# xuanyi-fu/xynet

Hardware: AMD Instinct MI355X
Metric: GiB/s device-resident WebSocket XOR-unmask, 64KiB frames, 1/2/4/8 GPUs (higher is better)
Workload: dtype u8; 1 GPU; config 3: 32768 x 64 KiB masked binary frames (H=14), one contiguous 2 GiB batch; decoder=lattice (k_stream_lattice), mode=fused (xyws_decode_stream: boundaries discovered on device), frames_per_gpu=32768, batch_bytes_per_gpu=2147942400, payload_bytes_per_gpu=2147483648, batch_copies=1, parallelism=shard-by-frame x1, no collective

## Files before the change

### xynet_amd/_lib.py

```python
import ctypes as C
import os
import re

PKG = os.path.dirname(os.path.abspath(__file__))
ROOT = os.path.dirname(PKG)
HEADER = os.path.join(ROOT, "include", "xyws.h")

XYWS_OK = 0
XYWS_ERR_DEVICE = -5
OPT_PARSE_ONLY = 0x1
OPT_UNMASKED_HINT = 0x2
OPT_SERIAL_SCAN = 0x4
OPT_WG256 = 0x8
OPT_TEST_LATSPEC = 0x10
OPT_TEST_LATDUMP = 0x20
OPT_LATX_NOWORK = 0x40
OPT_LATX_ONLY = 0x80
OPT_STATS = 0x100
OPT_SMALL_SEG = 0x200
OPT_LATTICE = 0x400
OPT_NO_LATDEC = 0x800
OPT_NO_DENSE0 = 0x1000
OPT_REDIRECT = 0x2000
OPT_NO_LATENTRY = 0x4000
OPT_WG1024 = 0x8000
OPT_RUNS_NOWAIT = 0x10000
OPT_NO_STORE = 0x20000
OPT_WG512 = 0x40000
OPT_DIAG = 0x80000
OPT_TEST_GIVEUP = 0x100000
OPT_NO_LATTICE = 0x200000
OPT_STEAL = 0x400000
OPT_TEST_STEAL = 0x800000
OPT_LAT_NOGATE = 0x1000000
OPT_LAT_GATE = 0x2000000
OPT_BIGSCAN = 0x4000000
OPT_LATX_NOCHK = 0x8000000
OPT_IOV_PIECES = 0x10000000
OPT_IOV_STAGE = 0x20000000
OPT_NO_BIGSCAN = 0x40000000
OPT_RUNS = 0x80000000
NSTATS = 48
ST_RUNS, ST_NONE, ST_BAD, ST_REPAIR, ST_CUT, ST_SPIN, ST_SEGS, ST_FRAMES = 0, 1, 2, 3, 4, 5, 6, 7
ST_P_WIN, ST_P_CAND, ST_P_UND, ST_P_TCOMP, ST_P_TCHECK, ST_P_TRES = 8, 9, 10, 11, 12, 13
ST_D_TENT, ST_D_TCHASE = 14, 15
ST_T_PRO, ST_T_MAIN, ST_T_WAIT, ST_T_FILL, ST_T_CHASE, ST_T_XOR = 16, 17, 18, 19, 20, 21
ST_T_TAIL, ST_T_PF, ST_T_CP = 22, 23, 24
ST_P_FILL, ST_P_SCAN, ST_P_PUB, ST_D_NOENT, ST_D_CHASE, ST_D_MISMATCH, ST_D_OVF = 25, 26, 27, 28, 29, 30, 31
ST_GIVEUP, ST_BRIDGE, ST_STEAL_REQ, ST_STEAL_ACC, ST_STEAL_SEGS = 32, 33, 34, 35, 36
ST_D_TVAL, ST_T_ROWS, ST_T_SER = 37, 38, 39
ST_P_LATTICE, ST_X_W0, ST_X_BITS, ST_X_SURV, ST_T_STRIDE = 40, 41, 42, 43, 46
LT_C_A, LT_C_C, LT_C_ADV, LT_D_FILL, LT_D_WB, LT_D_TAB, LT_D_WC = 16, 17, 18, 19, 20, 21, 22
LT_D_MASK, LT_D_WD, LT_D_ST, LT_D_WA, LT_SEGS, LT_GATE, LT_END = 23, 24, 25, 26, 27, 28, 29
R_WORDS = 32
R_H, R_W, R_S0, R_HEAD, R_OKW, R_HN, R_WN, R_CNT, R_TAIL, R_FIRST, R_F0 = 0, 1, 2, 7, 8, 9, 10, 11, 12, 13, 14
R_EFROM, R_ECNT, R_EORD, R_ECARRY, R_EP = 20, 21, 22, 23, 24
R_T0, R_T1, R_T2, R_SPLIT, R_XCC, R_NREC = 25, 26, 27, 28, 29, 30
POL_EPOCH, POL_BYTES, POL_FSMIN, POL_FSMAX, POL_DECODER, POL_WORDS = 0, 1, 2, 3, 4, 5
DEC_RUNS, DEC_RUNS512, DEC_LATTICE = 0, 2, 3
DERR_TABLE, DERR_TIMEOUT, DERR_STALE, DERR_TAG, DERR_SRC_OOB, DERR_ORPHANS = 0x1, 0x2, 0x4, 0x8, 0x100, 0x200
ERRORS = {-1: "invalid argument", -2: "HIP runtime error", -3: "device allocation failed",
          -4: "scratch capacity exceeded", -5: "device-side error", -6: "not complete yet"}


class XywsError(RuntimeError):
    def __init__(self, code, what=""):
        self.code = code
        super().__init__(f"xyws error {code} ({ERRORS.get(code, '?')}){': ' + what if what else ''}")


class Frame(C.Structure):
    _fields_ = [("frame_off", C.c_int64), ("payload_off", C.c_int64),
                ("payload_len", C.c_uint64), ("key", C.c_uint8 * 4),
                ("flags", C.c_uint8), ("hdr_len", C.c_uint8),
                ("status", C.c_uint8), ("reserved", C.c_uint8)]


class Carry(C.Structure):
    _fields_ = [("payload_remaining", C.c_uint64), ("phase", C.c_uint64),
                ("frames_total", C.c_uint64), ("key", C.c_uint8 * 4),
                ("hdr_len", C.c_uint8), ("hdr", C.c_uint8 * 14),
                ("reserved", C.c_uint8 * 21)]


class Verdict(C.Structure):
    _fields_ = [("close_code", C.c_uint16), ("peer_code", C.c_uint16), ("action", C.c_uint8),
                ("reserved", C.c_uint8 * 3)]


class Message(C.Structure):
    _fields_ = [("first_frame", C.c_uint64), ("nframes", C.c_uint64), ("out_off", C.c_uint64),
                ("length", C.c_uint64), ("status", C.c_uint32), ("opcode", C.c_uint8),
                ("reserved", C.c_uint8 * 3)]


class MsgCarry(C.Structure):
    _fields_ = [("length", C.c_uint64), ("nframes", C.c_uint64), ("first_frame", C.c_uint64),
                ("frame_remaining", C.c_uint64), ("frames_seen", C.c_uint64), ("status", C.c_uint32),
                ("opcode", C.c_uint8), ("frame_member", C.c_uint8), ("utf8_len", C.c_uint8),
                ("utf8", C.c_uint8 * 3), ("reserved", C.c_uint8 * 14)]


class ArenaResult(C.Structure):
    _fields_ = [("seq", C.c_uint64), ("offset", C.c_uint64), ("len", C.c_uint64), ("nframes", C.c_uint64),
                ("frames", C.POINTER(Frame)), ("carry", Carry)]

# ... 155 lines not shown
```

### xynet_amd/csrc/xyws_lattice.h

```cpp

constexpr uint64_t LAT_FMIN = 128;
constexpr uint64_t LAT_FMAX = 1ull << 40;
enum { LS_AGG = 1, LS_BRK = 3 };
constexpr uint32_t LAT_SLIST = 512;
constexpr uint32_t LAT_NOCLAIM = 0x7FFFFFFFu;
enum : uint64_t { RD_DONE = 0, RD_FULL = 1, RD_FROM = 2 };

template <uint32_t NT_, uint32_t SEG_>
struct lgeom {
  static constexpr uint32_t NT = NT_, SEG = SEG_;
  static constexpr uint32_t TMAX = SEG_ / LAT_FMIN + 3;
};
using G_LAT = lgeom<1024, 15 * 8 * 1024>;
using G_LAT5 = lgeom<1024, 15 * 5 * 1024>;
constexpr uint64_t LAT5_MIN_FRAME = 16384;
using G_LAT_SMALL = lgeom<64, 1024>;


template <class GA, class GB>
struct llay {
  static_assert(GA::NT == GB::NT, "one workgroup size");
  static constexpr uint32_t NT = GA::NT;
  static constexpr uint32_t SEG = GA::SEG > GB::SEG ? GA::SEG : GB::SEG;
  static constexpr uint32_t TMAX = GA::TMAX > GB::TMAX ? GA::TMAX : GB::TMAX;
};
template <class GL>
struct __attribute__((aligned(256))) lat_lds {
  cstate S0;
  uint64_t E, X0, F, kmax, c0, kbf, nseg;
  uint64_t gk;
  uint32_t na, cur, nxt, brk, quit, done_last, nsl, big, nogate;
  uint64_t sl_seg[LAT_SLIST], sl_k[LAT_SLIST];
  uint4 tab[GL::TMAX];
  alignas(256) uint8_t seg[GL::SEG + 48];
};

XYWS_DEV uint32_t lat_rel(uint64_t x, uint64_t ss) {
  if (x <= ss) return 0;
  const uint64_t d = x - ss;
  return d > 0xFFFFFFFFull ? 0xFFFFFFFFu : (uint32_t)d;
}

constexpr uint32_t LAT_GRP = 64;
XYWS_DEV uint64_t lat_grp_size(const run_params& P, uint64_t g) {
  const uint64_t a = g * LAT_GRP;
  return a >= P.nseg ? 0 : (P.nseg - a < LAT_GRP ? P.nseg - a : LAT_GRP);
}

XYWS_DEV uint64_t lat_advance(const run_params& P, uint64_t E, uint32_t lane) {
  const uint64_t w = uniform64(st_load(P.lat + LW_W));
  if (w >= P.nseg) return w;
  uint64_t w1 = w;
  {
    const uint64_t g0 = w / LAT_GRP, g = g0 + lane, gs = lat_grp_size(P, g);
    const bool full = !gs || st_load(P.lgrp + g) == gs;
    const uint64_t nf = __ballot(!full);
    const uint32_t c = nf ? (uint32_t)__builtin_ctzll(nf) : 64u;
    const uint64_t wg = (g0 + c) * LAT_GRP;
    if (wg > w1) w1 = wg < P.nseg ? wg : P.nseg;
  }
  if (w1 < P.nseg) {
    bool dec[4];
#pragma unroll
    for (uint32_t r = 0; r < 4; r++) {
      const uint64_t j = w1 + 4 * lane + r;
      dec[r] = j >= P.nseg || (st_load(P.lat + LW_STAT + j) >> 2) == E;
    }
    const uint32_t lc = !dec[0] ? 0u : !dec[1] ? 1u : !dec[2] ? 2u : !dec[3] ? 3u : 4u;
    const uint64_t nd = __ballot(lc < 4);
    uint64_t w2 = w1 + 256;
    if (nd) {
      const uint32_t f = (uint32_t)__builtin_ctzll(nd);
      w2 = w1 + 4 * f + (uint32_t)__shfl((int)lc, (int)f, 64);
    }
    w1 = w2 < P.nseg ? w2 : P.nseg;
  }
  if (w1 > w && lane == 0) __hip_atomic_fetch_max(P.lat + LW_W, w1, __ATOMIC_RELAXED, __HIP_MEMORY_SCOPE_AGENT);
  return w1;
}
XYWS_DEV void lat_wait_decided(const run_params& P, uint64_t E, uint64_t s, uint32_t lane) {
  for (uint32_t it = 0; lat_advance(P, E, lane) <= s; it++) {
    if (it >= (1u << 20)) {
      if (lane == 0) atomicOr(head_error(P), DERR_TIMEOUT);
      return;
    }
    __builtin_amdgcn_s_sleep(8);
  }
}

XYWS_DEV u32x4 lat_mask(const uint4* tab, uint32_t nent, uint32_t idx, uint32_t a) {
  const uint4 g = tab[idx];
  if (g.x <= a && a + 16u <= g.y) return u32x4{g.z, g.z, g.z, g.z};
  u32x4 m = span_key16(a, g.x, g.y, g.z);
  if (idx + 1 < nent) {
    const uint4 n = tab[idx + 1];
    if (n.x < a + 16u) m |= span_key16(a, n.x, n.y, n.z);
  }
  return m;
}

XYWS_DEV hdr_info lat_hdr(const run_params& P, const uint8_t* seg, uint32_t xr, uint64_t x) {
  const uint32_t* q = reinterpret_cast<const uint32_t*>(seg + (xr & ~3u));
  const uint32_t sh = xr & 3u, r0 = q[0], r1 = q[1], r2 = q[2], r3 = q[3], r4 = q[4];
  uint32_t w[4];
  w[0] = __builtin_amdgcn_alignbyte(r1, r0, sh);
  w[1] = __builtin_amdgcn_alignbyte(r2, r1, sh);
  w[2] = __builtin_amdgcn_alignbyte(r3, r2, sh);
  w[3] = __builtin_amdgcn_alignbyte(r4, r3, sh);
  const uint64_t room = P.hi - x;
  return parse_header_words(w, room < 16 ? (uint32_t)room : 16u);
}

XYWS_DEV __amdgpu_buffer_rsrc_t lat_rsrc(const run_params& P, uint64_t ss, uint32_t n) {
  const uint64_t top = (P.hi + 15) & ~15ull;
  const uint64_t room = top > ss ? top - ss : 0;
  return __builtin_amdgcn_make_buffer_rsrc(P.base + ss, 0, room < n ? (uint32_t)room : n, 0x00020000);
}

XYWS_DEV void write_frame(const run_params& P, uint64_t ord, uint64_t start, const hdr_info& h, uint64_t ps,
                          int32_t hdr_shift);

XYWS_DEV void lat_carried_frame(const run_params& P, const xyws_carry* cz) {
  if (!P.frames || !P.cap || cz->payload_remaining || !cz->hdr_len) return;
  const hdr_info hh = header_carried(P, cz);
  if (hh.hlen) write_frame(P, 0, P.lo, hh, P.lo + (hh.hlen - cz->hdr_len), (int32_t)cz->hdr_len);
}

template <class LL>
XYWS_DEV void lat_finish(const run_params& P, LL& L) {
  uint64_t* rd = P.lat + LW_REDIR;
  const xyws_carry* cz = P.cin_user ? P.cin_user : &k_zero_carry;
  {
    const uint32_t w = L.na == 2 ? LW_NBAIL_POL : L.na ? LW_NBAIL_HYP : L.big ? LW_NLOOP_A : LW_NLOOP_B;
    st_store(P.lat + w, st_load(P.lat + w) + 1);
  }
  if (L.na) {
    st_store(rd, RD_FULL);
  } else {
    const uint64_t b = st_load(P.lat + LW_BRK);
    const uint64_t X0 = L.X0, F = L.F, kmax = L.kmax, c0 = L.c0;
    lat_carried_frame(P, cz);
    if (b) {
      const uint64_t kb = ~b;
      const uint64_t tb = c0 + kb;
      uint64_t* rc = P.lat + LW_RCARRY;
#pragma unroll
      for (int i = 0; i < 8; i++) st_store(rc + i, 0);
      st_store(rc + 2, cz->frames_total + tb);
      st_store(rd + 1, X0 + kb * F);
      st_store(rd + 2, tb);
      st_store(rd, RD_FROM);
    } else {
      const uint64_t xl = X0 + (kmax - 1) * F;
      const hdr_info h = hdr_global(P, xl, NONE);
      uint64_t total = c0 + kmax;
      cstate S;
      if (!h.hlen) {
        S.X = xl; S.cov_ps = xl; S.cov_start = xl; S.cov_kw = 0; S.cov_key = 0; S.st = S_PARTIAL | S_NOCOV; S.pad = 0;
        total--;
      } else {
        S = frame_state(xl, h);
      }
      xyws_carry cinc;
#pragma unroll
      for (int i = 0; i < 8; i++) reinterpret_cast<uint64_t*>(&cinc)[i] = reinterpret_cast<const uint64_t*>(cz)[i];
      write_outputs(P, &cinc, total, S);
      dpol_publish(P, F, DEC_LATTICE);
      if (P.pol) {
        const uint64_t v[5] = {L.E, P.hi - P.lo, F, F, DEC_LATTICE};
#pragma unroll
        for (int i = 1; i < 5; i++) __hip_atomic_store(P.pol + i, v[i], __ATOMIC_RELAXED, __HIP_MEMORY_SCOPE_SYSTEM);
        __hip_atomic_store(P.pol, v[0], __ATOMIC_RELEASE, __HIP_MEMORY_SCOPE_SYSTEM);
      }
      st_store(rd, RD_DONE);
    }
  }
  uint32_t* cnt = reinterpret_cast<uint32_t*>(P.lat + LW_CNT);
  st_store(P.lat + LW_BRK, 0);
  st_store(P.lat + LW_W, 0);
  st_store(P.lat + LW_LOOPS, 0);
  __hip_atomic_store(cnt, 0u, __ATOMIC_RELAXED, __HIP_MEMORY_SCOPE_AGENT);
  __hip_atomic_store(cnt + 1, 0u, __ATOMIC_RELAXED, __HIP_MEMORY_SCOPE_AGENT);
  st_store(P.lat + LW_EPOCH, L.E);
}

XYWS_DEV bool lat_redirect(run_params& P) {
  if (!(P.opts & XYWS_OPT_REDIRECT)) return true;
  const uint64_t* r = P.lat + LW_REDIR;
  const uint64_t st = uniform64(st_load(r));
  if (st == RD_DONE) return false;
  if (st != RD_FROM) return true;
  const uint64_t p = uniform64(st_load(r + 1)), tb = uniform64(st_load(r + 2));
  const uint64_t pal = p & ~15ull;
  P.obias = p - P.lo;
  P.base += pal;
  P.lo = p - pal;
  P.hi -= pal;
  const uint64_t seg = P.segb, nseg = (P.hi + seg - 1) / seg, maxr = P.nruns;
  P.rbytes = nseg <= maxr ? seg : ((P.hi + maxr - 1) / maxr + 15) & ~15ull;
  P.nruns = (uint32_t)((P.hi + P.rbytes - 1) / P.rbytes);
  P.nflat = 2 * P.nruns;
  P.cin_user = reinterpret_cast<const xyws_carry*>(P.lat + LW_RCARRY);
  P.tbias = tb;
  if (P.frames) {
    const uint64_t c = P.cap < tb ? P.cap : tb;
    P.frames += c;
    P.cap -= c;
  }
  return true;
}

template <class G>
struct lat_io {
  static constexpr bool CTRL = G::NT >= 256;
  static constexpr uint32_t NW = G::NT / 64, NDW = CTRL ? NW - 1 : NW;
  static constexpr uint32_t NROW = G::SEG / 1024, K = (NROW + NDW - 1) / NDW;
  static constexpr uint32_t CLAIM = CTRL ? 64u : 0u;
  static_assert(G::SEG % 1024 == 0, "segments are whole 1 KiB rows");
  XYWS_DEV static bool data_wave(uint32_t wave) { return !CTRL || wave != 0; }
  XYWS_DEV static uint32_t row(uint32_t wave, uint32_t k) { return (CTRL ? wave - 1 : wave) + NDW * k; }
  XYWS_DEV static bool valid(uint32_t wave, uint32_t k) { return K * NDW == NROW || row(wave, k) < NROW; }
};

XYWS_DEV uint64_t lat_load_late(const uint64_t* p) {
  uint64_t v;
  asm volatile("global_load_dwordx2 %0, %1, off sc1" : "=v"(v) : "v"(p) : "memory");
  return v;
}

constexpr uint32_t LAT_NREP = 64, LAT_REPW = 32;
inline constexpr uint64_t lat_rep_off(uint64_t segs) {
  return (LW_STAT + segs + segs / 64 + 1 + LAT_REPW - 1) / LAT_REPW * LAT_REPW;
}
inline constexpr uint64_t lat_sl_off(uint64_t segs) { return lat_rep_off(segs) + LAT_NREP * LAT_REPW; }
XYWS_DEV void lat_raise_brk(const run_params& P, uint64_t k, uint32_t lane) {
  uint64_t o = 0;
// ... 61 lines not shown
  constexpr uint32_t CW = IO::CLAIM / 64u;
  auto issue = [&](uint32_t s, bool claim, bool rows) {
    if constexpr (DT) {
      if (wave == CW) {
        if (lane == 0) {
          if (claim)
            asm volatile("global_atomic_add %0, %1, %2, off sc0" : "=v"(ahead) : "v"(cnt), "v"(1u) : "memory");
          else
            ahead = LAT_NOCLAIM;
        }
        cx = lat_ctrl_load(P, s, G::SEG, X0, F, kmax, tid);
      }
      if (rows) {
        const __amdgpu_buffer_rsrc_t rs = lat_rsrc(P, (uint64_t)s * G::SEG, G::SEG);
#pragma unroll
        for (uint32_t k = 0; k < IO::K; k++)
          e[k] = __builtin_amdgcn_raw_buffer_load_b128(rs, IO::valid(wave, k) ? lane * 16u : OOB,
                                                       IO::row(wave, k) * 1024u, AUX_NT);
      }
    }
  };
  if (DT && cur != NONE32) {
    const uint32_t a0 = ahead;
    issue(cur, false, true);
    ahead = a0;
    const __amdgpu_buffer_rsrc_t rs = lat_rsrc(P, (uint64_t)cur * G::SEG, G::SEG);
#pragma unroll
    for (uint32_t k = 0; k < IO::K; k++)
      __builtin_amdgcn_raw_buffer_store_b128(u32x4{0u, 0u, 0u, 0u}, rs, OOB, k * 1024u, AUX_ST_STREAM);
  }
  const uint32_t dl = IO::CTRL ? tid - 64u : tid, NDL = IO::NDW * 64u;
  while (cur != NONE32) {
    asm volatile("" : "+v"(tid));
    const uint64_t ss = (uint64_t)cur * G::SEG;
    const uint64_t se = ss + G::SEG;
    const uint64_t ka = ss <= X0 ? 0 : (ss - X0 + F - 1) / F;
    clk.mark(cl ? LT_C_ADV : LT_D_ST);
    __syncthreads();
    clk.mark(cl ? LT_C_ADV : LT_D_WA);
    if constexpr (DT) {
#pragma unroll
      for (uint32_t k = 0; k < IO::K; k++)
        if (IO::valid(wave, k)) *reinterpret_cast<u32x4*>(&L.seg[IO::row(wave, k) * 1024u + lane * 16u]) = e[k];
      if (clk.on) asm volatile("s_waitcnt lgkmcnt(0)" ::: "memory");
    }
    if (DT && wave == CW) {
      asm volatile("" : "+v"(ahead), "+v"(cx) : "v"(e[IO::K - 1].x));
      const uint32_t ln = tid & 63u;
      if (ln < 9) *reinterpret_cast<uint32_t*>(&L.seg[G::SEG + 4u * ln]) = cx;
      if (lane == 0) {
        const uint32_t a = ahead + 2u * gridDim.x;
        L.nxt = a < P.nseg ? a : NONE32;
        L.brk = NONE32;
      }
    }
    clk.mark(cl ? LT_C_A : LT_D_FILL);
    __syncthreads();
    clk.mark(cl ? LT_C_A : LT_D_WB);
    const uint32_t nxt = uniform32(L.nxt);
    uint64_t kz = se <= X0 ? 0 : (se - X0 + F - 1) / F;
    if (kz > kmax) kz = kmax;
    const uint32_t nl = kz > ka ? (uint32_t)(kz - ka) : 0u;
    if constexpr (DT) {
      if (tid == IO::CLAIM) {
        uint4 c = {0u, 0u, 0u, 0u};
        if (ka == 0) {
          const cstate S0 = L.S0;
          if (!(S0.st & S_NOCOV)) c = uint4{lat_rel(S0.cov_ps, ss), lat_rel(X0, ss), S0.cov_kw, 0u};
        } else if (ka <= kmax) {
          const uint64_t xc = X0 + (ka - 1) * F;
          const uint32_t sh = (uint32_t)(xc & 3);
          uint32_t w[4];
          const uint32_t* cw = reinterpret_cast<const uint32_t*>(&L.seg[G::SEG + 16]);
#pragma unroll
          for (int i = 0; i < 4; i++) w[i] = __builtin_amdgcn_alignbyte(cw[i + 1], cw[i], sh);
          const uint64_t room = P.hi - xc;
          const hdr_info h = parse_header_words(w, room < 16 ? (uint32_t)room : 16u);
          if (h.hlen) {
            const uint64_t ps = xc + h.hlen;
            const uint64_t end = ka == kmax ? sat_add(ps, h.plen) : xc + F;
            c = uint4{lat_rel(ps, ss), lat_rel(end < P.hi ? end : P.hi, ss), aligned_key(h.key, ps, 0), 0u};
          }
        }
        L.tab[0] = c;
      }
      if (nxt != NONE32) issue(nxt, !L.quit, true);
      const uint32_t nlw = (P.opts & XYWS_OPT_LATX_NOWORK) ? 0u : nl;
      for (uint32_t i = dl; i < nlw; i += NDL) {
        const uint64_t k = ka + i;
        const uint64_t x = X0 + k * F;
        const uint32_t xr = (uint32_t)(x - ss);
        const hdr_info h = lat_hdr(P, L.seg, xr, x);
        const bool last = k + 1 == kmax;
        const uint64_t fend = h.hlen ? sat_add(x + h.hlen, h.plen) : x;
        const bool ok = h.hlen ? ((uint64_t)h.hlen + h.plen == F && h.plen < F) || (last && fend >= P.hi) : last;
        if (!ok) atomicMin(&L.brk, i);
        uint4 en = {xr, xr, 0u, 0u};
        if (h.hlen) {
          const uint64_t ps = x + h.hlen;
          en = uint4{lat_rel(ps, ss), lat_rel(fend < P.hi ? fend : P.hi, ss), aligned_key(h.key, ps, 0), 0u};
        }
        L.tab[1 + i] = en;
      }
    }
    if (CT && tid == 0) {
      asm volatile("s_waitcnt vmcnt(0)" : "+v"(brk_seen)::"memory");
      if (cl) clk.mark(LT_GATE);
      L.gk = brk_seen;
    }
    clk.mark(cl ? LT_C_A : LT_D_TAB);
    __syncthreads();
    clk.mark(cl ? LT_C_C : LT_D_WC);
    const uint32_t brk = uniform32(L.brk);
    const bool blind = (P.opts & XYWS_OPT_TEST_LATSPEC) != 0;
    const bool gate = it == 0 && !blind && !(P.opts & XYWS_OPT_LAT_NOGATE);
    if (CT && tid < 64) {
      const uint64_t gk = uniform64(L.gk);
      if (brk != NONE32 && !(gk && ~gk <= ka + brk)) lat_raise_brk(P, ka + brk, lane);
      if (tid == 0) {
        st_store(P.lat + LW_STAT + cur, (E << 2) | (brk != NONE32 ? LS_BRK : LS_AGG));
        __hip_atomic_fetch_add(P.lgrp + cur / LAT_GRP, 1ull, __ATOMIC_RELAXED, __HIP_MEMORY_SCOPE_AGENT);
      }
      if (gate) {
        const uint64_t tg = clk.on ? __builtin_amdgcn_s_memtime() : 0;
        lat_wait_decided(P, E, cur, lane);
        if (tg && tid == 0) stat_add(P, LT_END, __builtin_amdgcn_s_memtime() - tg);
        if (tid == 0) L.gk = st_load(P.lat + LW_BRK);
      }
      if (tid == 0) brk_seen = lat_load_late(P.lbrk + LAT_REPW * (blockIdx.x % LAT_NREP));
    }
    if (gate) __syncthreads();
    clk.mark(cl ? LT_C_C : LT_D_WD);
    const uint64_t b = blind ? 0 : uniform64(L.gk);
    uint64_t kst = brk != NONE32 ? ka + brk : kz;
    if (b && ~b < kst) kst = ~b;
    uint32_t stop = kst >= kz ? G::SEG : lat_rel(X0 + kst * F, ss);
    if (stop > G::SEG) stop = G::SEG;
    bool quit = b || brk != NONE32;
    if (stop && !gate) {
      if (nsl < LAT_SLIST) {
        if (tid == IO::CLAIM) {
          L.sl_seg[nsl] = cur;
          L.sl_k[nsl] = kst;
        }
        nsl++;
      } else {
        const uint64_t k0 = ka ? ka - 1 : 0;
        if (tid == IO::CLAIM)
          for (uint32_t r = 0; r <= LAT_NREP; r++)
            __hip_atomic_fetch_max(r < LAT_NREP ? P.lbrk + LAT_REPW * r : P.lat + LW_BRK, ~k0, __ATOMIC_RELAXED,
                                   __HIP_MEMORY_SCOPE_AGENT);
        if (k0 < kst) {
          stop = lat_rel(X0 + k0 * F, ss);
          kst = k0;
        }
        quit = true;
      }
    }
    if (quit && tid == IO::CLAIM) L.quit = 1;
    if constexpr (DT) {
      const uint32_t xka = ka < kmax ? lat_rel(X0 + ka * F, ss) : 0xFFFFFFFFu;
      const uint32_t nent = brk != NONE32 ? 1u + brk : 1u + nl;
      const uint32_t lo_r = lat_rel(P.lo, ss), hi_r = P.hi - ss < G::SEG ? (uint32_t)(P.hi - ss) : G::SEG;
      const __amdgpu_buffer_rsrc_t rs = lat_rsrc(P, ss, G::SEG);
      const bool any = !(P.opts & XYWS_OPT_NO_STORE);
      const bool work = !(P.opts & XYWS_OPT_LATX_NOWORK);
      uint32_t edge = 0;
      u32x4 dprev = {0u, 0u, 0u, 0u};
#pragma unroll
      for (uint32_t k = 0; k < IO::K; k++) {
        const bool ok = IO::valid(wave, k);
        const uint32_t a = (ok ? IO::row(wave, k) : 0u) * 1024u + lane * 16u;
        u32x4 d = *reinterpret_cast<const u32x4*>(&L.seg[a]);
        uint32_t idx = 0;
// ... 75 lines not shown
        const cstate S0 = L.S0;
        if (!(S0.st & S_NOCOV)) en = uint4{lat_rel(S0.cov_ps, ss), lat_rel(X0, ss), S0.cov_kw, 0u};
      } else if (g < kst && g < kmax) {
        const uint64_t x = X0 + g * F;
        const hdr_info h = hdr_global(P, x, NONE);
        if (h.hlen) {
          const uint64_t ps = x + h.hlen;
          const uint64_t end = g + 1 == kmax ? sat_add(ps, h.plen) : x + F;
          en = uint4{lat_rel(ps, ss), lat_rel(end < P.hi ? end : P.hi, ss), aligned_key(h.key, ps, 0), 0u};
        }
      }
      m |= span_key16(a, en.x, en.y, en.z);
    }
    if (a >= from && a >= lo_r && a + 16u <= top) {
      uint32_t* q = reinterpret_cast<uint32_t*>(P.base + ss + a);
      const uint32_t mm[4] = {m.x, m.y, m.z, m.w};
#pragma unroll
      for (int i = 0; i < 4; i++) {
        if (!mm[i]) continue;
        const uint32_t v = __hip_atomic_load(q + i, __ATOMIC_RELAXED, __HIP_MEMORY_SCOPE_AGENT);
        __hip_atomic_store(q + i, v ^ mm[i], __ATOMIC_RELAXED, __HIP_MEMORY_SCOPE_AGENT);
      }
      continue;
    }
#pragma unroll
    for (uint32_t b = 0; b < 16; b++) {
      const uint32_t y = a + b;
      const uint32_t mw = b < 4 ? m.x : b < 8 ? m.y : b < 12 ? m.z : m.w;
      const uint8_t kbyte = (uint8_t)(mw >> (8u * (b & 3u)));
      if (kbyte && y >= from && y >= lo_r && y < top) {
        uint8_t* q = P.base + ss + y;
        const uint8_t v = __hip_atomic_load(q, __ATOMIC_RELAXED, __HIP_MEMORY_SCOPE_AGENT);
        __hip_atomic_store(q, (uint8_t)(v ^ kbyte), __ATOMIC_RELAXED, __HIP_MEMORY_SCOPE_AGENT);
      }
    }
  }
}

constexpr uint32_t LAT_UNDO_POLLS = 2048;

template <class G, class LL>
XYWS_DEV void lat_body(const run_params& P, LL& L, uint32_t tid, uint32_t ahead) {
  using IO = lat_io<G>;
  uint32_t* cnt = reinterpret_cast<uint32_t*>(P.lat + LW_CNT);
  if (!L.na) {
    if constexpr (IO::CTRL) {
      if (__builtin_amdgcn_readfirstlane(tid >> 6) == 0)
        lat_loop<G, LR_CTRL>(P, L, tid, ahead);
      else
        lat_loop<G, LR_DATA>(P, L, tid, ahead);
    } else {
      lat_loop<G, LR_ALL>(P, L, tid, ahead);
    }
    __syncthreads();
    if (tid < 64) {
      uint64_t b = 0;
      if (tid == 0) __hip_atomic_fetch_add(P.lat + LW_LOOPS, 1ull, __ATOMIC_RELAXED, __HIP_MEMORY_SCOPE_AGENT);
      if (L.quit && L.nsl) {
        const uint32_t polls = (P.opts & XYWS_OPT_TEST_LATDUMP) ? 0u : LAT_UNDO_POLLS;
        bool ended = false;
        for (uint32_t it = 0; it < polls; it++) {
          if (uniform64(st_load(P.lat + LW_LOOPS)) >= gridDim.x) {
            ended = true;
            break;
          }
          __builtin_amdgcn_s_sleep(8);
        }
        if (ended) b = uniform64(st_load(P.lat + LW_BRK));
      }
      if (tid == 0) L.kbf = b && L.nsl ? ~b : NONE;
    }
    __syncthreads();
    const uint64_t kb = L.kbf;
    if (kb != NONE) {
      const uint32_t n = L.nsl;
      for (uint32_t j = 0; j < n; j++)
        if (kb < L.sl_k[j]) lat_undo<G>(P, L, tid, L.sl_seg[j], L.sl_k[j], kb);
      asm volatile("s_waitcnt vmcnt(0)" ::: "memory");
      __syncthreads();
      if (tid == 0) L.nsl = 0;
      __syncthreads();
    }
    lat_dump_list<G>(P, L, tid);
  }
  asm volatile("s_waitcnt vmcnt(0)" ::: "memory");
  __syncthreads();
  if (tid == 0) {
    __builtin_amdgcn_fence(__ATOMIC_RELEASE, "agent");
    asm volatile("s_waitcnt vmcnt(0)" ::: "memory");
    const uint32_t last = atomicAdd(cnt + 1, 1u) + 1 == gridDim.x ? 1u : 0u;
    if (last) {
      __builtin_amdgcn_fence(__ATOMIC_ACQUIRE, "agent");
      asm volatile("s_waitcnt vmcnt(0)" ::: "memory");
    }
    L.done_last = last;
  }
  __syncthreads();
  if (!L.done_last) return;
  if (tid == 0) {
    const uint64_t b = st_load(P.lat + LW_BRK);
    L.kbf = b && !L.na ? ~b : NONE;
  }
  __syncthreads();
  const uint64_t kb = L.kbf;
  if (kb != NONE) {
    if (tid == 0) L.nsl = 0;
    __syncthreads();
    for (uint32_t w = tid; w < gridDim.x; w += G::NT) {
      const uint64_t* q = P.lsl + (uint64_t)w * LAT_LSW;
      const uint32_t n = (uint32_t)st_load(q);
      for (uint32_t i = 0; i < n; i++) {
        const uint64_t kst = st_load(q + 2 + 2 * i);
        if (kb < kst) {
          const uint32_t j = atomicAdd(&L.nsl, 1u);
          if (j < LAT_SLIST) {
            L.sl_seg[j] = st_load(q + 1 + 2 * i);
            L.sl_k[j] = kst;
          }
        }
      }
    }
    __syncthreads();
    const uint32_t nu = L.nsl;
    if (nu <= LAT_SLIST) {
      for (uint32_t j = 0; j < nu; j++) lat_undo<G>(P, L, tid, L.sl_seg[j], L.sl_k[j], kb);
    } else {
      for (uint32_t w = 0; w < gridDim.x; w++) {
        const uint64_t* q = P.lsl + (uint64_t)w * LAT_LSW;
        const uint32_t n = (uint32_t)st_load(q);
        for (uint32_t i = 0; i < n; i++) {
          const uint64_t kst = st_load(q + 2 + 2 * i);
          if (kb < kst) lat_undo<G>(P, L, tid, st_load(q + 1 + 2 * i), kst, kb);
        }
      }
    }
    asm volatile("s_waitcnt vmcnt(0)" ::: "memory");
    __syncthreads();
  }
  for (uint64_t g = tid; g * LAT_GRP < P.nseg; g += G::NT)
    __hip_atomic_store(P.lgrp + g, 0ull, __ATOMIC_RELAXED, __HIP_MEMORY_SCOPE_AGENT);
  if (tid < LAT_NREP) __hip_atomic_store(P.lbrk + LAT_REPW * tid, 0ull, __ATOMIC_RELAXED, __HIP_MEMORY_SCOPE_AGENT);
  if (tid != 0) return;
  lat_finish(P, L);
}

template <class GA, class GB>
__global__ void __launch_bounds__(GB::NT)
__attribute__((amdgpu_waves_per_eu(GB::NT >= 256 ? GB::NT / 256 : 1))) k_stream_lattice(run_params P0) {
  using GL = llay<GA, GB>;
  using IO = lat_io<GB>;
  static_assert(lat_io<GA>::CLAIM == IO::CLAIM, "one claim lane");
  extern __shared__ __attribute__((aligned(256))) uint8_t xs_lds[];
  lat_lds<GL>& L = *reinterpret_cast<lat_lds<GL>*>(xs_lds);
  const uint32_t tid = threadIdx.x;
  uint32_t ahead = NONE32;
  if (tid == 0) {
    const xyws_carry* cz = P0.cin_user ? P0.cin_user : &k_zero_carry;
    carry_words cc;
    uint32_t r0[5];
    uint64_t dp, ep;
    {
      u32x4 g;
      asm volatile("global_load_dwordx4 %0, %1, off sc1" : "=v"(g) : "v"(P0.lat + LW_DPOL) : "memory");
#pragma unroll
      for (int i = 0; i < 8; i++) cc.w[i] = reinterpret_cast<const uint64_t*>(cz)[i];
      const uint64_t a0 = P0.lo & ~3ull, dl = (P0.hi + 3) & ~3ull;
#pragma unroll
      for (int i = 0; i < 5; i++) {
        const uint64_t q = a0 + 4 * i;
        r0[i] = *reinterpret_cast<const uint32_t*>(P0.base + (q < dl ? q : dl - 4));
      }
      asm volatile("s_waitcnt vmcnt(0)" : "+v"(g)::"memory");
#pragma unroll
      for (int i = 0; i < 5; i++)
        if (a0 + 4 * i >= dl) r0[i] = 0u;
      dp = (uint64_t)g.x | ((uint64_t)g.y << 32);
      ep = (uint64_t)g.z | ((uint64_t)g.w << 32);
    }
    L.E = ep + 1;
    const bool dvalid = dp >> 63, dreg = (dp & ((1ull << 48) - 1)) >= LAT_FMIN;
    const uint64_t ddec = (dp >> 48) & 0x7Fu;
    uint32_t na = dvalid && !dreg && !(P0.opts & XYWS_OPT_LATTICE) ? 2u : 0u;
    L.nogate = dvalid && dreg && ddec == DEC_LATTICE && !(P0.opts & XYWS_OPT_LAT_GATE) ? 1u : 0u;
    uint64_t c0 = 0;
    const cstate S0 = initial_state_w(P0, cc, c0);
    if (!na && ((S0.st & S_PARTIAL) || S0.X >= P0.hi)) na = 1u;
    uint64_t F = 0, kmax = 0;
    if (!na) {
      hdr_info h;
      if (S0.X == P0.lo) {
        const uint32_t sh = (uint32_t)(P0.lo & 3);
        uint32_t w[4];
#pragma unroll
        for (int i = 0; i < 4; i++) w[i] = __builtin_amdgcn_alignbyte(r0[i + 1], r0[i], sh);
        const uint64_t room = P0.hi - P0.lo;
        h = parse_header_words(w, room < 16 ? (uint32_t)room : 16u);
      } else {
        h = hdr_global(P0, S0.X, NONE);
      }
      F = sat_add(h.hlen, h.plen);
      if (!h.hlen || F < LAT_FMIN || F > LAT_FMAX) na = 1;
      else kmax = (P0.hi - S0.X + F - 1) / F;
    }
    if (!na && kmax > 1 && !(P0.opts & (XYWS_OPT_TEST_LATSPEC | XYWS_OPT_LATX_NOCHK))) {
      const uint64_t dl = (P0.hi + 3) & ~3ull;
      uint32_t r[2][5];
#pragma unroll
      for (int j = 0; j < 2; j++) {
        const uint64_t a = (S0.X + (j + 1) * F) & ~3ull;
#pragma unroll
        for (int i = 0; i < 5; i++) {
          const uint64_t q = a + 4 * i;
          r[j][i] = (j == 0 || kmax > 2) && q < dl ? *reinterpret_cast<const uint32_t*>(P0.base + q) : 0u;
        }
      }
#pragma unroll
      for (int j = 0; j < 2; j++) {
        const uint64_t k = j + 1;
        if (k >= kmax) break;
        const uint64_t x = S0.X + k * F;
        const uint32_t sh = (uint32_t)(x & 3);
        uint32_t w[4];
#pragma unroll
        for (int i = 0; i < 4; i++) w[i] = __builtin_amdgcn_alignbyte(r[j][i + 1], r[j][i], sh);
        const uint64_t room = P0.hi - x;
        const hdr_info h = parse_header_words(w, room < 16 ? (uint32_t)room : 16u);
        const bool last = k + 1 == kmax;
        const uint64_t fend = h.hlen ? sat_add(x + h.hlen, h.plen) : x;
        const bool ok = h.hlen ? ((uint64_t)h.hlen + h.plen == F && h.plen < F) || (last && fend >= P0.hi) : last;
        if (!ok) na = 1;
      }
    }
    const bool big = GA::SEG != GB::SEG && !na && F >= LAT5_MIN_FRAME;
    const uint64_t seg = big ? GA::SEG : GB::SEG;
    const uint64_t nseg = (P0.hi + seg - 1) / seg;
    L.nseg = nseg;
    L.S0 = S0;
    L.c0 = c0;
    L.X0 = S0.X;
    L.F = F;
    L.kmax = kmax;
    L.na = na;
    L.quit = 0;
    L.nsl = 0;
    L.big = big ? 1u : 0u;
    L.cur = !na && blockIdx.x < nseg ? blockIdx.x : NONE32;
  }
  if (tid == IO::CLAIM) ahead = blockIdx.x - gridDim.x;
  __syncthreads();
  run_params P = P0;
  P.nseg = uniform64(L.nseg);
  P.opts &= ~XYWS_OPT_LAT_NOGATE;
  if (uniform32(L.nogate)) P.opts |= XYWS_OPT_LAT_NOGATE;
  if constexpr (GA::SEG != GB::SEG) {
    if (uniform32(L.big)) {
      lat_body<GA>(P, L, tid, ahead);
      return;
    }
  }
  lat_body<GB>(P, L, tid, ahead);
}
```

### xynet_amd/csrc/xyws_stream.h

```cpp
#pragma once
#include <hip/hip_runtime.h>
#include <stdint.h>
#include "xyws.h"
#include "xyws_host.h"


constexpr uint32_t HEAD_TICKET = 0;
constexpr uint32_t HEAD_ERROR = 4;
constexpr uint32_t HEAD_TOTAL = 8;
constexpr uint32_t HEAD_EPOCH = 16;
constexpr uint32_t HEAD_CARRY = 64;
constexpr uint32_t HEAD_STATS = 128;
constexpr uint32_t XYWS_NSTATS = 48;
constexpr uint32_t HW_DONE = 512;
constexpr uint32_t HW_BAD = 520;
constexpr uint32_t HW_TOTAL = 528;
constexpr uint32_t HW_FINAL = 536;
constexpr uint32_t HW_EMIT_SLOW = 584;
constexpr uint32_t HW_EMIT_FLAG = 592;
constexpr uint32_t HW_FSMAX = 600;
constexpr uint32_t HW_FSMIN = 608;
constexpr uint32_t HW_DPOL = 616;
constexpr uint32_t HEAD_BYTES = 1024;
static_assert(HEAD_CARRY + 64 <= HEAD_STATS && HEAD_STATS + 8 * XYWS_NSTATS <= HW_DONE, "head areas overlap");
// ... 13 lines not shown
  R_HEAD = 7,
  R_OKW = 8,
  R_HN = 9,
  R_WN = 10,
  R_CNT = 11,
  R_TAIL = 12,
  R_FIRST = 13,
  R_F0 = 14,
  R_EFROM = 20,
  R_ECNT = 21,
  R_EORD = 22,
  R_ECARRY = 23,
  R_EP = 24,
  R_T0 = 25,
  R_T1 = 26,
  R_T2 = 27,
  R_SPLIT = 28,
  R_XCC = 29,
  R_NREC = 30,
  R_WORDS = 32
};
static_assert(R_S0 + 5 == R_HEAD && R_F0 + 5 < R_EFROM && R_NREC < R_WORDS, "run record words overlap");

struct run_layout {
  uint64_t granules, split, prog, records;
  uint64_t zeroed, total;
};
inline run_layout run_layout_of(uint64_t units) {
  const auto pad = [](uint64_t bytes) { return (bytes + 255) & ~255ull; };
  run_layout l;
  l.granules = HEAD_BYTES;
  l.split = l.granules + pad(32 * units);
  l.prog = l.split + pad(16 * units);
  l.records = l.prog + pad(8 * units);
  l.zeroed = l.records;
  l.total = l.records + 2 * units * R_WORDS * 8;
  return l;
}

enum {
  LW_CNT = 0,
  LW_BRK = 2,
  LW_UNMASK = 3,
  LW_W = 4,
  LW_LOOPS = 5,
  LW_DPOL = 6,
  LW_EPOCH = 7,
  LW_REDIR = 8,
  LW_NBAIL_POL = 12,
  LW_NBAIL_HYP = 13,
  LW_NLOOP_A = 14,
  LW_NLOOP_B = 15,
  LW_RCARRY = 16,
  LW_STAT = 32
};
static_assert(LW_EPOCH == LW_DPOL + 1 && LW_DPOL % 2 == 0, "one 16-byte granule");

enum {
  ST_RUNS = 0,
  ST_NONE = 1,
  ST_BAD = 2,
  ST_REPAIR = 3,
  ST_CUT = 4,
  ST_SPIN = 5,
  ST_SEGS = 6,
  ST_FRAMES = 7,
  ST_P_WIN = 8,
  ST_P_CAND = 9,
  ST_P_UND = 10,
  ST_P_TCOMP = 11,
  ST_P_TCHECK = 12,
  ST_P_TRES = 13,
  ST_D_TENT = 14,
  ST_D_TCHASE = 15,
  ST_T_PRO = 16,
  LT_C_A = 16,
  ST_T_MAIN = 17,
  LT_C_C = 17,
  ST_T_WAIT = 18,
  LT_C_ADV = 18,
  ST_T_FILL = 19,
  LT_D_FILL = 19,
  ST_T_CHASE = 20,
  LT_D_WB = 20,
  ST_T_XOR = 21,
  LT_D_TAB = 21,
  ST_T_TAIL = 22,
  LT_D_WC = 22,
  ST_T_PF = 23,
  LT_D_MASK = 23,
  ST_T_CP = 24,
  LT_D_WD = 24,
  ST_P_FILL = 25,
  LT_D_ST = 25,
  ST_P_SCAN = 26,
  LT_D_WA = 26,
  ST_P_PUB = 27,
  LT_SEGS = 27,
  ST_D_NOENT = 28,
  LT_GATE = 28,
  ST_D_CHASE = 29,
  LT_END = 29,
  ST_D_MISMATCH = 30,
  ST_D_OVF = 31,
  ST_GIVEUP = 32,
  ST_BRIDGE = 33,
  ST_STEAL_REQ = 34,
  ST_STEAL_ACC = 35,
  ST_STEAL_SEGS = 36,
  ST_D_TVAL = 37,
  ST_T_ROWS = 38,
  ST_T_SER = 39,
  ST_P_LATTICE = 40,
  ST_X_W0 = 41,
  ST_X_BITS = 42,
  ST_X_SURV = 43,
  ST_T_STRIDE = 46
};
enum {
  LCLK_SLOT0 = 16,
  LCLK_NSLOTS = 16
};
static_assert(LT_C_A == LCLK_SLOT0 && LT_END < LCLK_SLOT0 + LCLK_NSLOTS && LCLK_SLOT0 + LCLK_NSLOTS <= ST_GIVEUP,
              "the lattice's clocks stay in the shared slots");
static_assert(ST_T_STRIDE < XYWS_NSTATS, "a stats slot outside the head's stats area");

enum {
  POL_EPOCH = 0,
  POL_BYTES = 1,
  POL_FSMIN = 2,
  POL_FSMAX = 3,
  POL_DECODER = 4,
  POL_WORDS = 5
};
enum : uint64_t {
  DEC_RUNS = 0,
  DEC_RUNS512 = 2,
  DEC_LATTICE = 3
};

constexpr uint64_t SCRATCH_MIN_RUNS = 64, SCRATCH_MIN_SEGS = 64;
struct stream_scratch {
  xyws_internal::dev_area runs;
  int ncu = 256;
  xyws_internal::dev_area desc;
  volatile uint64_t* pol_h = nullptr;
  uint64_t* pol_d = nullptr;
  xyws_internal::dev_area lat;
};

void stream_scratch_init(stream_scratch* s, int device);
void stream_scratch_free(stream_scratch* s);
int stream_scratch_reserve(stream_scratch* s, uint64_t max_batch_bytes, uint64_t max_frames);
uint32_t stream_scratch_error(stream_scratch* s, bool clear);
int stream_scratch_stats(stream_scratch* s, uint64_t out[XYWS_NSTATS]);
int64_t stream_scratch_records(stream_scratch* s, uint64_t* out, uint64_t max_runs);
int stream_scratch_lattice(stream_scratch* s, uint64_t out[5]);
int stream_scratch_unmask_counter(stream_scratch* s, bool capturing, uint32_t** out);

#define XYWS_OPT_WG256 0x8u
#define XYWS_OPT_TEST_LATSPEC 0x10u
#define XYWS_OPT_TEST_LATDUMP 0x20u
#define XYWS_OPT_LATX_NOWORK 0x40u
#define XYWS_OPT_LATX_ONLY 0x80u
#define XYWS_OPT_STATS 0x100u
#define XYWS_OPT_SMALL_SEG 0x200u
#define XYWS_OPT_LATTICE 0x400u
#define XYWS_OPT_NO_LATDEC 0x800u
#define XYWS_OPT_NO_DENSE0 0x1000u
// ... 65 lines not shown
```

Baseline: 3075 GiB/s.

## Precompute last-frame carry state in segment workers to shorten lattice finish tail

The workgroup that handles the final segment now computes the last frame's carry state and writes it to a new tail record in scratch, tagged with the epoch. The finishing block loads the break word, the tail record and the input carry in one batch of loads. This lets it skip the global header re-read on its serial critical path, and the carried-frame write and outputs are moved after the bookkeeping stores. The atomic add for the loop counter and a reordered policy load trim a few more serialized round trips, at the cost of extra LDS state and a fallback path when the epoch tag does not match.

```diff
diff --git a/xynet_amd/_lib.py b/xynet_amd/_lib.py
--- a/xynet_amd/_lib.py
+++ b/xynet_amd/_lib.py
@@ -52,6 +52,7 @@
 ST_P_LATTICE, ST_X_W0, ST_X_BITS, ST_X_SURV, ST_T_STRIDE = 40, 41, 42, 43, 46
 LT_C_A, LT_C_C, LT_C_ADV, LT_D_FILL, LT_D_WB, LT_D_TAB, LT_D_WC = 16, 17, 18, 19, 20, 21, 22
 LT_D_MASK, LT_D_WD, LT_D_ST, LT_D_WA, LT_SEGS, LT_GATE, LT_END = 23, 24, 25, 26, 27, 28, 29
+LT_TAIL, LT_TAIL_FIN = 44, 45
 R_WORDS = 32
 R_H, R_W, R_S0, R_HEAD, R_OKW, R_HN, R_WN, R_CNT, R_TAIL, R_FIRST, R_F0 = 0, 1, 2, 7, 8, 9, 10, 11, 12, 13, 14
 R_EFROM, R_ECNT, R_EORD, R_ECARRY, R_EP = 20, 21, 22, 23, 24
diff --git a/xynet_amd/csrc/xyws_lattice.h b/xynet_amd/csrc/xyws_lattice.h
--- a/xynet_amd/csrc/xyws_lattice.h
+++ b/xynet_amd/csrc/xyws_lattice.h
@@ -24,12 +24,20 @@
   static constexpr uint32_t SEG = GA::SEG > GB::SEG ? GA::SEG : GB::SEG;
   static constexpr uint32_t TMAX = GA::TMAX > GB::TMAX ? GA::TMAX : GB::TMAX;
 };
+struct lat_fin {
+  uint64_t brk;
+  uint64_t rec[8];
+  xyws_carry cin;
+};
 template <class GL>
 struct __attribute__((aligned(256))) lat_lds {
   cstate S0;
   uint64_t E, X0, F, kmax, c0, kbf, nseg;
   uint64_t gk;
+  uint64_t ttail, tfin;
+  lat_fin fin;
   uint32_t na, cur, nxt, brk, quit, done_last, nsl, big, nogate;
+  uint32_t lastp;
   uint64_t sl_seg[LAT_SLIST], sl_k[LAT_SLIST];
   uint4 tab[GL::TMAX];
   alignas(256) uint8_t seg[GL::SEG + 48];
@@ -126,52 +134,75 @@
   if (hh.hlen) write_frame(P, 0, P.lo, hh, P.lo + (hh.hlen - cz->hdr_len), (int32_t)cz->hdr_len);
 }
 
+XYWS_DEV cstate lat_last_state(uint64_t xl, const hdr_info& h, uint64_t c0, uint64_t kmax, uint64_t& total) {
+  total = c0 + kmax;
+  if (h.hlen) return frame_state(xl, h);
+  cstate S;
+  S.X = xl; S.cov_ps = xl; S.cov_start = xl; S.cov_kw = 0; S.cov_key = 0; S.st = S_PARTIAL | S_NOCOV; S.pad = 0;
+  total--;
+  return S;
+}
+
+XYWS_DEV void lat_tail_put(const run_params& P, uint64_t E, const cstate& S, uint64_t total) {
+  uint64_t* r = P.lat + LW_TAIL;
+  put_state(r + 1, S);
+  st_store(r + 6, total);
+  st_store(r, E);
+}
+
+XYWS_DEV void lat_finish_load(const run_params& P, lat_fin& f) {
+  const xyws_carry* cz = P.cin_user ? P.cin_user : &k_zero_carry;
+  uint64_t c[8];
+#pragma unroll
+  for (int i = 0; i < 8; i++) c[i] = reinterpret_cast<const uint64_t*>(cz)[i];
+  uint64_t b;
+  u32x4 t0, t1, t2, t3;
+  asm volatile(
+      "global_load_dwordx2 %0, %5, off sc1\n\t"
+      "global_load_dwordx4 %1, %6, off sc1\n\t"
+      "global_load_dwordx4 %2, %6, off offset:16 sc1\n\t"
+      "global_load_dwordx4 %3, %6, off offset:32 sc1\n\t"
+      "global_load_dwordx4 %4, %6, off offset:48 sc1\n\t"
+      "s_waitcnt vmcnt(0)"
+      : "=&v"(b), "=&v"(t0), "=&v"(t1), "=&v"(t2), "=&v"(t3)
+      : "v"(P.lat + LW_BRK), "v"(P.lat + LW_TAIL)
+      : "memory");
+  f.brk = b;
+  const u32x4 t[4] = {t0, t1, t2, t3};
+#pragma unroll
+  for (int i = 0; i < 4; i++) {
+    f.rec[2 * i] = (uint64_t)t[i].x | ((uint64_t)t[i].y << 32);
+    f.rec[2 * i + 1] = (uint64_t)t[i].z | ((uint64_t)t[i].w << 32);
+  }
+#pragma unroll
+  for (int i = 0; i < 8; i++) reinterpret_cast<uint64_t*>(&f.cin)[i] = c[i];
+}
+
 template <class LL>
 XYWS_DEV void lat_finish(const run_params& P, LL& L) {
   uint64_t* rd = P.lat + LW_REDIR;
-  const xyws_carry* cz = P.cin_user ? P.cin_user : &k_zero_carry;
+  const xyws_carry* cz = &L.fin.cin;
   {
     const uint32_t w = L.na == 2 ? LW_NBAIL_POL : L.na ? LW_NBAIL_HYP : L.big ? LW_NLOOP_A : LW_NLOOP_B;
-    st_store(P.lat + w, st_load(P.lat + w) + 1);
-  }
+    __hip_atomic_fetch_add(P.lat + w, 1ull, __ATOMIC_RELAXED, __HIP_MEMORY_SCOPE_AGENT);
+  }
+  bool held = false;
   if (L.na) {
     st_store(rd, RD_FULL);
   } else {
-    const uint64_t b = st_load(P.lat + LW_BRK);
-    const uint64_t X0 = L.X0, F = L.F, kmax = L.kmax, c0 = L.c0;
-    lat_carried_frame(P, cz);
+    const uint64_t b = L.fin.brk;
     if (b) {
       const uint64_t kb = ~b;
-      const uint64_t tb = c0 + kb;
+      const uint64_t tb = L.c0 + kb;
       uint64_t* rc = P.lat + LW_RCARRY;
 #pragma unroll
       for (int i = 0; i < 8; i++) st_store(rc + i, 0);
       st_store(rc + 2, cz->frames_total + tb);
-      st_store(rd + 1, X0 + kb * F);
+      st_store(rd + 1, L.X0 + kb * L.F);
       st_store(rd + 2, tb);
       st_store(rd, RD_FROM);
     } else {
-      const uint64_t xl = X0 + (kmax - 1) * F;
-      const hdr_info h = hdr_global(P, xl, NONE);
-      uint64_t total = c0 + kmax;
-      cstate S;
-      if (!h.hlen) {
-        S.X = xl; S.cov_ps = xl; S.cov_start = xl; S.cov_kw = 0; S.cov_key = 0; S.st = S_PARTIAL | S_NOCOV; S.pad = 0;
-        total--;
-      } else {
-        S = frame_state(xl, h);
-      }
-      xyws_carry cinc;
-#pragma unroll
-      for (int i = 0; i < 8; i++) reinterpret_cast<uint64_t*>(&cinc)[i] = reinterpret_cast<const uint64_t*>(cz)[i];
-      write_outputs(P, &cinc, total, S);
-      dpol_publish(P, F, DEC_LATTICE);
-      if (P.pol) {
-        const uint64_t v[5] = {L.E, P.hi - P.lo, F, F, DEC_LATTICE};
-#pragma unroll
-        for (int i = 1; i < 5; i++) __hip_atomic_store(P.pol + i, v[i], __ATOMIC_RELAXED, __HIP_MEMORY_SCOPE_SYSTEM);
-        __hip_atomic_store(P.pol, v[0], __ATOMIC_RELEASE, __HIP_MEMORY_SCOPE_SYSTEM);
-      }
+      held = true;
       st_store(rd, RD_DONE);
     }
   }
@@ -182,6 +213,39 @@
   __hip_atomic_store(cnt, 0u, __ATOMIC_RELAXED, __HIP_MEMORY_SCOPE_AGENT);
   __hip_atomic_store(cnt + 1, 0u, __ATOMIC_RELAXED, __HIP_MEMORY_SCOPE_AGENT);
   st_store(P.lat + LW_EPOCH, L.E);
+  if (!L.na) lat_carried_frame(P, cz);
+  if (held) {
+    const uint64_t F = L.F, kmax = L.kmax, c0 = L.c0;
+    uint64_t total;
+    cstate S;
+    if (L.fin.rec[0] == L.E) {
+      S.X = L.fin.rec[1];
+      S.cov_ps = L.fin.rec[2];
+      S.cov_start = L.fin.rec[3];
+      S.cov_kw = (uint32_t)L.fin.rec[4];
+      S.cov_key = (uint32_t)(L.fin.rec[4] >> 32);
+      S.st = (uint32_t)L.fin.rec[5];
+      S.pad = 0;
+      total = L.fin.rec[6];
+    } else {
+      const uint64_t xl = L.X0 + (kmax - 1) * F;
+      S = lat_last_state(xl, hdr_global(P, xl, NONE), c0, kmax, total);
+    }
+    write_outputs(P, cz, total, S);
+    dpol_publish(P, F, DEC_LATTICE);
+    if (P.pol) {
+      const uint64_t v[5] = {L.E, P.hi - P.lo, F, F, DEC_LATTICE};
+#pragma unroll
+      for (int i = 1; i < 5; i++) __hip_atomic_store(P.pol + i, v[i], __ATOMIC_RELAXED, __HIP_MEMORY_SCOPE_SYSTEM);
+      __hip_atomic_store(P.pol, v[0], __ATOMIC_RELEASE, __HIP_MEMORY_SCOPE_SYSTEM);
+    }
+  }
+  if (stats_on(P) && L.ttail) {
+    asm volatile("s_waitcnt vmcnt(0)" ::: "memory");
+    const uint64_t t = __builtin_amdgcn_s_memtime();
+    stat_add(P, LT_TAIL, t - L.ttail);
+    stat_add(P, LT_TAIL_FIN, t - L.tfin);
+  }
 }
 
 XYWS_DEV bool lat_redirect(run_params& P) {
@@ -349,6 +413,7 @@
         const uint32_t a = ahead + 2u * gridDim.x;
         L.nxt = a < P.nseg ? a : NONE32;
         L.brk = NONE32;
+        L.lastp = NONE32;
       }
     }
     clk.mark(cl ? LT_C_A : LT_D_FILL);
@@ -392,6 +457,7 @@
         const uint64_t fend = h.hlen ? sat_add(x + h.hlen, h.plen) : x;
         const bool ok = h.hlen ? ((uint64_t)h.hlen + h.plen == F && h.plen < F) || (last && fend >= P.hi) : last;
         if (!ok) atomicMin(&L.brk, i);
+        if (last && ok) L.lastp = xr;
         uint4 en = {xr, xr, 0u, 0u};
         if (h.hlen) {
           const uint64_t ps = x + h.hlen;
@@ -417,6 +483,13 @@
       if (tid == 0) {
         st_store(P.lat + LW_STAT + cur, (E << 2) | (brk != NONE32 ? LS_BRK : LS_AGG));
         __hip_atomic_fetch_add(P.lgrp + cur / LAT_GRP, 1ull, __ATOMIC_RELAXED, __HIP_MEMORY_SCOPE_AGENT);
+        const uint32_t lp = L.lastp;
+        if (lp != NONE32 && brk == NONE32) {
+          const uint64_t x = ss + lp;
+          uint64_t total;
+          const cstate S = lat_last_state(x, lat_hdr(P, L.seg, lp, x), L.c0, kmax, total);
+          lat_tail_put(P, E, S, total);
+        }
       }
       if (gate) {
         const uint64_t tg = clk.on ? __builtin_amdgcn_s_memtime() : 0;
@@ -598,6 +671,7 @@
     } else {
       lat_loop<G, LR_ALL>(P, L, tid, ahead);
     }
+    if (tid == 0 && stats_on(P)) L.ttail = __builtin_amdgcn_s_memtime();
     __syncthreads();
     if (tid < 64) {
       uint64_t b = 0;
@@ -644,7 +718,9 @@
   __syncthreads();
   if (!L.done_last) return;
   if (tid == 0) {
-    const uint64_t b = st_load(P.lat + LW_BRK);
+    if (stats_on(P)) L.tfin = __builtin_amdgcn_s_memtime();
+    lat_finish_load(P, L.fin);
+    const uint64_t b = L.fin.brk;
     L.kbf = b && !L.na ? ~b : NONE;
   }
   __syncthreads();
@@ -707,7 +783,6 @@
     uint64_t dp, ep;
     {
       u32x4 g;
-      asm volatile("global_load_dwordx4 %0, %1, off sc1" : "=v"(g) : "v"(P0.lat + LW_DPOL) : "memory");
 #pragma unroll
       for (int i = 0; i < 8; i++) cc.w[i] = reinterpret_cast<const uint64_t*>(cz)[i];
       const uint64_t a0 = P0.lo & ~3ull, dl = (P0.hi + 3) & ~3ull;
@@ -716,7 +791,10 @@
         const uint64_t q = a0 + 4 * i;
         r0[i] = *reinterpret_cast<const uint32_t*>(P0.base + (q < dl ? q : dl - 4));
       }
-      asm volatile("s_waitcnt vmcnt(0)" : "+v"(g)::"memory");
+      asm volatile("global_load_dwordx4 %0, %1, off sc1\n\ts_waitcnt vmcnt(0)"
+                   : "=&v"(g)
+                   : "v"(P0.lat + LW_DPOL)
+                   : "memory");
 #pragma unroll
       for (int i = 0; i < 5; i++)
         if (a0 + 4 * i >= dl) r0[i] = 0u;
@@ -789,6 +867,7 @@
     L.na = na;
     L.quit = 0;
     L.nsl = 0;
+    L.ttail = 0;
     L.big = big ? 1u : 0u;
     L.cur = !na && blockIdx.x < nseg ? blockIdx.x : NONE32;
   }
diff --git a/xynet_amd/csrc/xyws_stream.h b/xynet_amd/csrc/xyws_stream.h
--- a/xynet_amd/csrc/xyws_stream.h
+++ b/xynet_amd/csrc/xyws_stream.h
@@ -89,8 +89,10 @@
   LW_NLOOP_A = 14,
   LW_NLOOP_B = 15,
   LW_RCARRY = 16,
+  LW_TAIL = 24,
   LW_STAT = 32
 };
+static_assert(LW_RCARRY + 8 <= LW_TAIL && LW_TAIL % 2 == 0 && LW_TAIL + 8 <= LW_STAT, "the tail record's words");
 static_assert(LW_EPOCH == LW_DPOL + 1 && LW_DPOL % 2 == 0, "one 16-byte granule");
 
 enum {
@@ -152,6 +154,8 @@
   ST_X_W0 = 41,
   ST_X_BITS = 42,
   ST_X_SURV = 43,
+  LT_TAIL = 44,
+  LT_TAIL_FIN = 45,
   ST_T_STRIDE = 46
 };
 enum {
```

Result: no change. 3079 GiB/s, median of 6 (+0.1%).
